# gmongaras/Stable-Diffusion-3-From-Scratch

Hardware: AMD Instinct MI355X
Metric: train images/sec MMDiT-B 256^2 bf16 (higher is better)
Workload: dtype bf16

## Files before the change

### stable-diffusion-3-from-scratch_amd/csrc/attention.hip

```cpp
#include <type_traits>
#include "common.h"

namespace {

constexpr int HD = 64;
constexpr int KT = 64;
constexpr int P144 = 144;
constexpr int P192 = 192;
constexpr float LOG2E = 1.4426950408889634f;
constexpr float LN2 = 0.6931471805599453f;

__device__ __forceinline__ int acc_row(int r, int lane) { return (r & 3) + 8 * (r >> 2) + 4 * (lane >> 5); }

__device__ __forceinline__ bf16x8 pack_frag(const f32x16& p, int h8) {
  u32x4 w;
#pragma unroll
  for (int i = 0; i < 4; i++) w[i] = pack_bf2(p[h8 * 8 + 2 * i], p[h8 * 8 + 2 * i + 1]);
  return __builtin_bit_cast(bf16x8, w);
}

__device__ __forceinline__ bf16x8 tr_frag(const char* tile, int pitch, int rb, int h8, int cb, int lane) {
  const int row = rb + 16 * h8 + 4 * (lane >> 5) + ((lane & 15) >> 2);
  const int col = cb * 32 + 16 * ((lane >> 4) & 1) + (lane & 3) * 4;
  const char* p = tile + row * pitch + col * 2;
  s16x4 lo = lds_tr16(p), hi = lds_tr16(p + 8 * pitch);
  s16x8 r = {lo[0], lo[1], lo[2], lo[3], hi[0], hi[1], hi[2], hi[3]};
  return __builtin_bit_cast(bf16x8, r);
}

__device__ __forceinline__ bf16x8 row_frag(const char* tile, int pitch, int rb, int ks, int lane) {
  return *LDS_PTR(const bf16x8, tile + (rb + (lane & 31)) * pitch + (ks * 16 + (lane >> 5) * 8) * 2);
}

template <int NT> constexpr int tile_chunks() { return (512 + NT - 1) / NT; }
template <int NT>
__device__ __forceinline__ void tile_g2r(u32x4 (&st)[tile_chunks<NT>()], const bf16_t* g, int row0, int nrows_total, int tid) {
#pragma unroll
  for (int i = 0; i < tile_chunks<NT>(); i++) {
    const int c = tid + i * NT, row = c >> 3, kc = c & 7;
    st[i] = (c < 512 && row0 + row < nrows_total) ? *(const u32x4*)(g + (int64_t)(row0 + row) * HD + kc * 8) : (u32x4){0, 0, 0, 0};
  }
}
template <int NT>
__device__ __forceinline__ void tile_r2s(const u32x4 (&st)[tile_chunks<NT>()], char* tile, int pitch, int tid) {
#pragma unroll
  for (int i = 0; i < tile_chunks<NT>(); i++) {
    const int c = tid + i * NT, row = c >> 3, kc = c & 7;
    if (512 % NT == 0 || c < 512) *LDS_PTR(u32x4, tile + row * pitch + kc * 16) = st[i];
  }
}

__device__ __forceinline__ int sw2(int r) { return ((r >> 1) & 7) ^ (((r >> 1) & 1) << 2); }
template <int NT>
__device__ __forceinline__ void tile_r2s_sw(const u32x4 (&st)[tile_chunks<NT>()], char* tile, int tid) {
#pragma unroll
  for (int i = 0; i < tile_chunks<NT>(); i++) {
    const int c = tid + i * NT, row = c >> 3, kc = c & 7;
    if (512 % NT == 0 || c < 512) *LDS_PTR(u32x4, tile + row * 128 + ((kc ^ sw2(row)) << 4)) = st[i];
  }
}
__device__ __forceinline__ bf16x8 row_frag_d(const char* tile, int rb, int ks, int lane) {
  const int r = rb + (lane & 31);
  return *LDS_PTR(const bf16x8, tile + r * 128 + (((ks * 2 + (lane >> 5)) ^ sw2(r)) << 4));
}
__device__ __forceinline__ bf16x8 tr_frag_d(const char* tile, int rb, int h8, int cb, int lane) {
  const int row = rb + 16 * h8 + 4 * (lane >> 5) + ((lane & 15) >> 2);
  const int cbyte = (cb * 32 + 16 * ((lane >> 4) & 1) + (lane & 3) * 4) * 2;
  const char* p0 = tile + row * 128 + ((((cbyte >> 4) ^ sw2(row)) << 4) | (cbyte & 15));
  const char* p1 = tile + (row + 8) * 128 + ((((cbyte >> 4) ^ sw2(row + 8)) << 4) | (cbyte & 15));
  s16x4 lo = lds_tr16(p0), hi = lds_tr16(p1);
  s16x8 r = {lo[0], lo[1], lo[2], lo[3], hi[0], hi[1], hi[2], hi[3]};
  return __builtin_bit_cast(bf16x8, r);
}

__device__ __forceinline__ const bf16_t* tok_ptr(const bf16_t* x_img, const bf16_t* x_txt, int64_t b, int s, int n_img, int n_txt, int D, int h) {
  if (s < n_img) return x_img + ((b * n_img + s) * (int64_t)D + h * HD);
  return x_txt ? x_txt + ((b * n_txt + (s - n_img)) * (int64_t)D + h * HD) : nullptr;
}

__device__ __forceinline__ void map_block(int ntile, int BH, int& tile, int& bh) {
  const int id = blockIdx.x;
  if (BH % 8 == 0) {
    const int xcd = id & 7, j = id >> 3;
    tile = j % ntile;
    bh = (j / ntile) * 8 + xcd;
  } else {
    tile = id % ntile;
    bh = id / ntile;
  }
}

__device__ __forceinline__ float partner32(float x, int lane);
constexpr float QK_RMS_EPS = 1.1920929e-07f;

struct QkFuse {
  const bf16_t* qkv_x; const bf16_t* qkv_c;
  const float* wq_x; const float* wk_x; const float* wq_c; const float* wk_c;
  const float* rcos; const float* rsin;
  bf16_t* dqkv_x; bf16_t* dqkv_c;
  float* dw;
};

constexpr int QK_ROW_F = 68;
constexpr int QK_WAVE_BYTES = 32 * QK_ROW_F * 4;
template <int NW> constexpr int qk_lds_bytes() { return NW * QK_WAVE_BYTES + 128 * 4; }

__device__ __forceinline__ void acc_to_lds(const f32x16 (&acc)[2], float* tile, int lane) {
  float* p = tile + (lane & 31) * QK_ROW_F + 4 * (lane >> 5);
#pragma unroll
  for (int db = 0; db < 2; db++)
#pragma unroll
    for (int g = 0; g < 4; g++)
      *LDS_PTR(f32x4, p + db * 32 + 8 * g) = (f32x4){acc[db][g * 4], acc[db][g * 4 + 1], acc[db][g * 4 + 2], acc[db][g * 4 + 3]};
  __builtin_amdgcn_wave_barrier();
}
__device__ __forceinline__ void acc_to_lds_half(const f32x16 (&acc)[2], float* tile16, int lane, int half) {
  if (((lane & 31) >> 4) == half) {
    float* p = tile16 + (lane & 15) * QK_ROW_F + 4 * (lane >> 5);
#pragma unroll
    for (int db = 0; db < 2; db++)
#pragma unroll
      for (int g = 0; g < 4; g++)
        *LDS_PTR(f32x4, p + db * 32 + 8 * g) = (f32x4){acc[db][g * 4], acc[db][g * 4 + 1], acc[db][g * 4 + 2], acc[db][g * 4 + 3]};
  }
  __builtin_amdgcn_wave_barrier();
}
__device__ __forceinline__ void lds_row8(const float* tile, int r, int c, float (&v)[8]) {
  const f32x4 a = *LDS_PTR(const f32x4, tile + r * QK_ROW_F + 8 * c), b = *LDS_PTR(const f32x4, tile + r * QK_ROW_F + 8 * c + 4);
#pragma unroll
  for (int e = 0; e < 4; e++) { v[e] = a[e]; v[4 + e] = b[e]; }
}
__device__ __forceinline__ void qk_bwd_rows(u32x4 (&xr)[4], int lane, int nvalid, const bf16_t* x0, int64_t pitch) {
  const int c = lane & 7, rsub = lane >> 3;
#pragma unroll
  for (int it = 0; it < 4; it++) xr[it] = __builtin_nontemporal_load((const u32x4*)(x0 + min(it * 8 + rsub, nvalid - 1) * pitch + 8 * c));
}
template <int IT0 = 0, int IT1 = 4>
__device__ __forceinline__ void qk_bwd_tile(const float* tile, float mul, int lane, int nvalid, const bf16_t* x0, bf16_t* o0, int64_t pitch,
                                            const float* w, const float* cs0, const float* sn0, float* sdw, const u32x4* xpre = nullptr) {
  const int c = lane & 7, rsub = lane >> 3;
  float w8[8], dw[8];
  ld8(w + 8 * c, w8);
#pragma unroll
  for (int e = 0; e < 8; e++) dw[e] = 0.f;
  u32x4 xr[4];
  if (xpre) {
#pragma unroll
    for (int it = IT0; it < IT1; it++) xr[it] = xpre[it];
  } else {
#pragma unroll
    for (int it = IT0; it < IT1; it++) xr[it] = __builtin_nontemporal_load((const u32x4*)(x0 + min(it * 8 + rsub, nvalid - 1) * pitch + 8 * c));
  }
  const bool rope = cs0 != nullptr;
  const float* tc = rope ? cs0 : w;
  const float* ts = rope ? sn0 : w;
  auto body = [&](auto full_t) __attribute__((always_inline)) {
    constexpr bool FULL = decltype(full_t)::value;
    float c8[8], s8[8];
    auto request = [&](int it) __attribute__((always_inline)) {
      const int rq = rope ? (FULL ? it * 8 + rsub : min(it * 8 + rsub, nvalid - 1)) : 0;
      ld8(tc + rq * 64 + 8 * c, c8);
      ld8(ts + rq * 64 + 8 * c, s8);
    };
    request(IT0);
#pragma unroll
    for (int it = IT0; it < IT1; it++) {
      const int r = it * 8 + rsub;
      const bool valid = FULL || r < nvalid;
      float dz[8], x[8];
#pragma unroll
      for (int e = 0; e < 4; e++) { x[2 * e] = __builtin_bit_cast(float, xr[it][e] << 16); x[2 * e + 1] = __builtin_bit_cast(float, xr[it][e] & 0xffff0000u); }
      lds_row8(tile, r, c, dz);
#pragma unroll
      for (int e = 0; e < 8; e++) dz[e] *= mul;
      if (rope) {
#pragma unroll
        for (int p = 0; p < 4; p++) {
          const float da = dz[2 * p], dbv = dz[2 * p + 1];
          dz[2 * p] = da * c8[2 * p] + dbv * s8[2 * p + 1];
          dz[2 * p + 1] = dbv * c8[2 * p + 1] - da * s8[2 * p];
        }
      }
      if (it + 1 < IT1) request(it + 1);
      float ss = 0.f;
#pragma unroll
      for (int e = 0; e < 8; e++) ss += x[e] * x[e];
      const float rinv = rsqrtf(sum8(ss) * (1.f / 64.f) + QK_RMS_EPS);
      float dot = 0.f;
#pragma unroll
      for (int e = 0; e < 8; e++) {
        x[e] *= rinv;
        dw[e] += valid ? dz[e] * x[e] : 0.f;
        dz[e] *= w8[e];
        dot += dz[e] * x[e];
      }
      dot = sum8(dot) * (1.f / 64.f);
      float o[8];
#pragma unroll
      for (int e = 0; e < 8; e++) o[e] = rinv * (dz[e] - x[e] * dot);
      if (valid) st8(o0 + r * pitch + 8 * c, o);
    }
  };
  if (nvalid >= 8 * IT1) body(std::integral_constant<bool, true>{});
  else body(std::integral_constant<bool, false>{});
#pragma unroll
  for (int e = 0; e < 8; e++) {
    float v = dw[e];
    v += __shfl_xor(v, 8, 64);
    v += __shfl_xor(v, 16, 64);
    v += __shfl_xor(v, 32, 64);
    if (lane < 8) atomicAdd(&sdw[8 * c + e], v);
  }
}
template <int IT0 = 0, int IT1 = 4>
__device__ __forceinline__ void rows_from_tile(const float* tile, int lane, int nvalid, bf16_t* o0, int64_t pitch) {
  const int c = lane & 7, rsub = lane >> 3;
#pragma unroll
  for (int it = IT0; it < IT1; it++) {
    const int r = it * 8 + rsub;
    float v[8];
    lds_row8(tile, r, c, v);
    if (r < nvalid) st8(o0 + r * pitch + 8 * c, v);
  }
}

template <int NW, bool ORACLE>
__global__ __launch_bounds__(NW * 64) void attn_fwd_kernel(const bf16_t* __restrict__ Q, const bf16_t* __restrict__ K, const bf16_t* __restrict__ V,
                                                            int BH, int H, int S, int n_img, float scale,
                                                            bf16_t* __restrict__ Ox, bf16_t* __restrict__ Oc, float* __restrict__ lse) {
  constexpr int NT = NW * 64;
  __shared__ __attribute__((aligned(16))) char smem[2 * KT * P144 + 2 * KT * P192];
  auto kt = [&](int i) { return smem + i * KT * P144; };
  auto vt = [&](int i) { return smem + 2 * KT * P144 + i * KT * P192; };

  const int tid = threadIdx.x, lane = tid & 63, wave = tid >> 6;
  MMDIT_YOUNG_HALF_PRIO();
  int qtile, bh;
  map_block((S + 32 * NW - 1) / (32 * NW), BH, qtile, bh);
  const int h = bh % H;
  const int64_t b = bh / H;
  const bf16_t* Qb = Q + (int64_t)bh * S * HD;
  const bf16_t* Kb = K + (int64_t)bh * S * HD;
  const bf16_t* Vb = V + (int64_t)bh * S * HD;
// ... 535 lines not shown
  constexpr int NT = NW * 64;
  __shared__ __attribute__((aligned(16))) char smem_static[FUSE ? 16 : 2 * KT * 128 + 2 * KT * 4];
  extern __shared__ __attribute__((aligned(16))) char smem_dyn[];
  char* smem = FUSE ? smem_dyn : smem_static;
  char* qtile = smem;
  char* dotile = smem + KT * 128;
  float* lse_s = (float*)(smem + 2 * KT * 128);
  float* del_s = lse_s + KT;
  const int tid = threadIdx.x, lane = tid & 63, wave = tid >> 6;
  MMDIT_YOUNG_HALF_PRIO();
  int ktile, bh;
  map_block((S + 32 * NW - 1) / (32 * NW), BH, ktile, bh);
  const int h = bh % H;
  const int64_t b = bh / H;
  const bf16_t* Qb = Q + (int64_t)bh * S * HD;
  const bf16_t* Kb = K + (int64_t)bh * S * HD;
  const bf16_t* Vb = V + (int64_t)bh * S * HD;
  const int key = ktile * 32 * NW + wave * 32 + (lane & 31);
  const bool active = ktile * 32 * NW + wave * 32 < S;
  const int keyc = min(key, S - 1);
  const int n_txt = S - n_img, D = H * HD;

  bf16x8 kf[4], vf[4];
#pragma unroll
  for (int ks = 0; ks < 4; ks++) {
    kf[ks] = *(const bf16x8*)(Kb + (int64_t)keyc * HD + ks * 16 + (lane >> 5) * 8);
    vf[ks] = *(const bf16x8*)(Vb + (int64_t)keyc * HD + ks * 16 + (lane >> 5) * 8);
  }
  f32x16 dk[2], dv[2];
#pragma unroll
  for (int db = 0; db < 2; db++)
#pragma unroll
    for (int r = 0; r < 16; r++) { dk[db][r] = 0.f; dv[db][r] = 0.f; }

  const int nq = (S + KT - 1) / KT;
  u32x4 sq[tile_chunks<NT>()], sd[tile_chunks<NT>()];
  float lv = 0.f, dl = 0.f;
  auto request = [&](int jq) {
    tile_g2r<NT>(sq, Qb, jq * KT, S, tid);
#pragma unroll
    for (int i = 0; i < tile_chunks<NT>(); i++) {
      const int c = tid + i * NT, row = c >> 3, kc = c & 7, s = jq * KT + row;
      const bf16_t* p = (c < 512 && s < S) ? tok_ptr(dOx, dOc, b, s, n_img, n_txt, D, h) : nullptr;
      sd[i] = p ? *(const u32x4*)(p + kc * 8) : (u32x4){0, 0, 0, 0};
    }
    lv = 0.f, dl = 0.f;
    if (tid < KT && jq * KT + tid < S) { lv = lse[(int64_t)bh * S + jq * KT + tid]; dl = delta[(int64_t)bh * S + jq * KT + tid]; }
  };
  request(0);
  stamp();
  for (int jq = 0; jq < nq; jq++) {
    __syncthreads();
    stamp();
    tile_r2s_sw<NT>(sq, qtile, tid);
    tile_r2s_sw<NT>(sd, dotile, tid);
    if (tid < KT) { lse_s[tid] = lv * LOG2E; del_s[tid] = dl; }
    stamp();
    __syncthreads();
    stamp();
#ifndef MMDIT_DKV_NO_PREFETCH
    if (jq + 1 < nq) request(jq + 1);
#endif
    if (active) {
#pragma unroll
    for (int qb = 0; qb < 2; qb++) {
      if (jq * KT + qb * 32 >= S) continue;
      f32x16 s, dp;
#pragma unroll
      for (int r = 0; r < 16; r++) { s[r] = 0.f; dp[r] = 0.f; }
#pragma unroll
      for (int ks = 0; ks < 4; ks++) {
        s = __builtin_amdgcn_mfma_f32_32x32x16_bf16(row_frag_d(qtile, qb * 32, ks, lane), kf[ks], s, 0, 0, 0);
        dp = __builtin_amdgcn_mfma_f32_32x32x16_bf16(row_frag_d(dotile, qb * 32, ks, lane), vf[ks], dp, 0, 0, 0);
      }
      if constexpr (TRACE) stamp();
      f32x16 ds;
#pragma unroll
      for (int g = 0; g < 4; g++) {
        const int r0 = qb * 32 + 8 * g + 4 * (lane >> 5);
        const f32x4 l4 = *LDS_PTR(const f32x4, lse_s + r0);
        const f32x4 d4 = *LDS_PTR(const f32x4, del_s + r0);
#pragma unroll
        for (int e = 0; e < 4; e++) {
          const int r = g * 4 + e;
          const float p = fast_exp2(fmaf(s[r], scale * LOG2E, -l4[e]));
          s[r] = p;
          ds[r] = p * (dp[r] - d4[e]);
        }
      }
      if ((jq + 1) * KT > S) {
#pragma unroll
        for (int g = 0; g < 4; g++)
#pragma unroll
          for (int e = 0; e < 4; e++)
            if (jq * KT + qb * 32 + 8 * g + 4 * (lane >> 5) + e >= S) { s[g * 4 + e] = 0.f; ds[g * 4 + e] = 0.f; }
      }
      if constexpr (TRACE) stamp();
#pragma unroll
      for (int h8 = 0; h8 < 2; h8++) {
        const bf16x8 pf = pack_frag(s, h8), dsf = pack_frag(ds, h8);
#pragma unroll
        for (int db = 0; db < 2; db++) {
          dv[db] = __builtin_amdgcn_mfma_f32_32x32x16_bf16(tr_frag_d(dotile, qb * 32, h8, db, lane), pf, dv[db], 0, 0, 0);
          dk[db] = __builtin_amdgcn_mfma_f32_32x32x16_bf16(tr_frag_d(qtile, qb * 32, h8, db, lane), dsf, dk[db], 0, 0, 0);
        }
      }
      if constexpr (TRACE) stamp();
    }
    }
    if constexpr (TRACE) { const int done = !active ? 0 : (jq * KT + 32 >= S ? 1 : 2); for (int i = done * 3; i < 6; i++) stamp(); }
#ifdef MMDIT_DKV_NO_PREFETCH
    if (jq + 1 < nq) request(jq + 1);
#endif
  }
  stamp();
  if constexpr (FUSE) {
    const int k0 = ktile * 32 * NW + wave * 32;
    const bool img = k0 < n_img;
    const int tok0 = img ? k0 : k0 - n_img, nvalid = min(32, (img ? n_img : S) - k0);
    const int64_t pitch = 3 * (int64_t)D, off = (img ? b * n_img + tok0 : b * n_txt + tok0) * pitch + D + h * HD;
    u32x4 xk[4];
    if (active) qk_bwd_rows(xk, lane, nvalid, (img ? F.qkv_x : F.qkv_c) + off, pitch);
    __syncthreads();
    float* sdw = (float*)(smem + NW * QK_WAVE_BYTES);
    if (tid < 128) sdw[tid] = 0.f;
    __syncthreads();
    if (active) {
      bf16_t* ob = (img ? F.dqkv_x : F.dqkv_c) + off;
      float* tile = (float*)(smem + wave * QK_WAVE_BYTES);
      acc_to_lds(dk, tile, lane);
      qk_bwd_tile(tile, scale, lane, nvalid, (img ? F.qkv_x : F.qkv_c) + off, ob, pitch, img ? F.wk_x : F.wk_c,
                  img ? F.rcos + (int64_t)tok0 * 64 : nullptr, img ? F.rsin + (int64_t)tok0 * 64 : nullptr, sdw + (img ? 0 : 64), xk);
      __builtin_amdgcn_wave_barrier();
      acc_to_lds(dv, tile, lane);
      rows_from_tile(tile, lane, nvalid, ob + D, pitch);
    }
    __syncthreads();
    if (tid < 128 && sdw[tid] != 0.f) atomicAdd(F.dw + (tid >> 6) * 128 + 64 + (tid & 63), sdw[tid]);
  } else if (key < S) {
    TG* pk = dK + ((int64_t)bh * S + key) * HD;
    TG* pv = dV + ((int64_t)bh * S + key) * HD;
#pragma unroll
    for (int db = 0; db < 2; db++)
#pragma unroll
      for (int g = 0; g < 4; g++) {
        float k4[4] = {dk[db][g * 4] * scale, dk[db][g * 4 + 1] * scale, dk[db][g * 4 + 2] * scale, dk[db][g * 4 + 3] * scale};
        float v4[4] = {dv[db][g * 4], dv[db][g * 4 + 1], dv[db][g * 4 + 2], dv[db][g * 4 + 3]};
        st4(pk + db * 32 + 8 * g + 4 * (lane >> 5), k4);
        st4(pv + db * 32 + 8 * g + 4 * (lane >> 5), v4);
      }
  }
  if constexpr (TRACE) asm volatile("s_waitcnt vmcnt(0)" ::: "memory");
  stamp();
}

#ifdef MMDIT_PROBES
constexpr int OP_MAXB = 13;
constexpr int OP_DST = 80;
constexpr int OP_DQ_BYTES = OP_MAXB * QK_WAVE_BYTES;
constexpr int OP_R_DST0 = 2 * KT * 128 + 2 * KT * 4;
constexpr int OP_R_BYTES = OP_R_DST0 + 8 * 32 * OP_DST;
constexpr int OP_LDS = OP_DQ_BYTES + OP_R_BYTES + 256 * 4;

__global__ __launch_bounds__(512) void attn_bwd_onepass_kernel(const bf16_t* __restrict__ Q, const bf16_t* __restrict__ K, const bf16_t* __restrict__ V,
                                                               const bf16_t* __restrict__ Ox, const bf16_t* __restrict__ Oc,
                                                               const bf16_t* __restrict__ dOx, const bf16_t* __restrict__ dOc, const float* __restrict__ lse,
                                                               int BH, int H, int S, int n_img, float scale, QkFuse F, int dbg) {
  constexpr int NT = 512;
  extern __shared__ __attribute__((aligned(16))) char smem_dyn[];
  float* dqa = (float*)smem_dyn;
  char* R = smem_dyn + OP_DQ_BYTES;
  char* qtile = R;
  char* dotile = R + KT * 128;
  float* lse_s = (float*)(R + 2 * KT * 128);
  float* del_s = lse_s + KT;
  float* sdw = (float*)(smem_dyn + OP_DQ_BYTES + OP_R_BYTES);
  const int tid = threadIdx.x, lane = tid & 63, wave = __builtin_amdgcn_readfirstlane(tid >> 6);
  char* dst_w = R + OP_R_DST0 + wave * (32 * OP_DST);
  int tile0, bh;
  map_block(1, BH, tile0, bh);
  const int h = bh % H;
  const int64_t b = bh / H;
  const bf16_t* Qb = Q + (int64_t)bh * S * HD;
  const bf16_t* Kb = K + (int64_t)bh * S * HD;
  const bf16_t* Vb = V + (int64_t)bh * S * HD;
  const int n_txt = S - n_img, D = H * HD;
  const int64_t pitch = 3 * (int64_t)D;
  const int nkb = (S + 31) >> 5, nq = (S + KT - 1) / KT;

  for (int i = tid; i < OP_DQ_BYTES / 16; i += NT) *LDS_PTR(f32x4, dqa + 4 * i) = (f32x4){0.f, 0.f, 0.f, 0.f};
  if (tid < 256) sdw[tid] = 0.f;

  u32x4 sq[1], sd[1], so[1];
  float lv = 0.f;
  auto request = [&](int jq) {
    tile_g2r<NT>(sq, Qb, jq * KT, S, tid);
    const int row = tid >> 3, kc = tid & 7, sidx = jq * KT + row;
    const bf16_t* pd = sidx < S ? tok_ptr(dOx, dOc, b, sidx, n_img, n_txt, D, h) : nullptr;
    const bf16_t* po = sidx < S ? tok_ptr(Ox, Oc, b, sidx, n_img, n_txt, D, h) : nullptr;
    sd[0] = pd ? *(const u32x4*)(pd + kc * 8) : (u32x4){0, 0, 0, 0};
    so[0] = (pd && po) ? *(const u32x4*)(po + kc * 8) : (u32x4){0, 0, 0, 0};
    lv = 0.f;
    if (tid < KT && jq * KT + tid < S) lv = lse[(int64_t)bh * S + jq * KT + tid];
  };

#pragma unroll 1
  for (int pass = 0; pass * 8 < nkb; pass++) {
    const int kblk = pass * 8 + wave;
    const bool active = kblk < nkb;
    const int key = kblk * 32 + (lane & 31), keyc = min(key, S - 1);
    const bool ragged_keys = kblk * 32 + 32 > S;
    __syncthreads();
    bf16x8 kf[4], vf[4], kt[2][2];
#pragma unroll
    for (int ks = 0; ks < 4; ks++) {
      kf[ks] = *(const bf16x8*)(Kb + (int64_t)keyc * HD + ks * 16 + (lane >> 5) * 8);
      vf[ks] = *(const bf16x8*)(Vb + (int64_t)keyc * HD + ks * 16 + (lane >> 5) * 8);
    }
    {
      char* kw = R + wave * 4096;
#pragma unroll
      for (int i = 0; i < 4; i++) {
        const int c = lane + 64 * i, row = c >> 3, kc = c & 7;
        const u32x4 v = *(const u32x4*)(Kb + (int64_t)min(kblk * 32 + row, S - 1) * HD + kc * 8);
        *LDS_PTR(u32x4, kw + row * 128 + ((kc ^ sw2(row)) << 4)) = v;
      }
      __builtin_amdgcn_wave_barrier();
#pragma unroll
      for (int h8 = 0; h8 < 2; h8++)
#pragma unroll
        for (int db = 0; db < 2; db++) kt[h8][db] = tr_frag_d(kw, 0, h8, db, lane);
    }
    f32x16 dk[2], dv[2];
#pragma unroll
    for (int db = 0; db < 2; db++)
#pragma unroll
      for (int r = 0; r < 16; r++) { dk[db][r] = 0.f; dv[db][r] = 0.f; }
    request(0);
#pragma unroll 1
    for (int jq = 0; jq < nq; jq++) {
      __syncthreads();
      tile_r2s_sw<NT>(sq, qtile, tid);
      tile_r2s_sw<NT>(sd, dotile, tid);
      {
        float dl = 0.f;
#pragma unroll
        for (int e = 0; e < 4; e++)
          dl += __builtin_bit_cast(float, so[0][e] << 16) * __builtin_bit_cast(float, sd[0][e] << 16) +
                __builtin_bit_cast(float, so[0][e] & 0xffff0000u) * __builtin_bit_cast(float, sd[0][e] & 0xffff0000u);
        dl = sum8(dl);
        if ((tid & 7) == 0) del_s[tid >> 3] = dl;
      }
      if (tid < KT) lse_s[tid] = lv * LOG2E;
      __syncthreads();
      if (jq + 1 < nq) request(jq + 1);
      if (active) {
#pragma unroll 1
        for (int qb = 0; qb < 2; qb++) {
          if (jq * KT + qb * 32 >= S) continue;
          f32x16 sacc, dp;
#pragma unroll
          for (int r = 0; r < 16; r++) { sacc[r] = 0.f; dp[r] = 0.f; }
#pragma unroll
          for (int ks = 0; ks < 4; ks++) {
            sacc = __builtin_amdgcn_mfma_f32_32x32x16_bf16(row_frag_d(qtile, qb * 32, ks, lane), kf[ks], sacc, 0, 0, 0);
            dp = __builtin_amdgcn_mfma_f32_32x32x16_bf16(row_frag_d(dotile, qb * 32, ks, lane), vf[ks], dp, 0, 0, 0);
          }
          f32x16 ds;
#pragma unroll
          for (int g = 0; g < 4; g++) {
            const int r0 = qb * 32 + 8 * g + 4 * (lane >> 5);
            const f32x4 l4 = *LDS_PTR(const f32x4, lse_s + r0);
            const f32x4 d4 = *LDS_PTR(const f32x4, del_s + r0);
#pragma unroll
            for (int e = 0; e < 4; e++) {
              const int r = g * 4 + e;
              const float pe = fast_exp2(fmaf(sacc[r], scale * LOG2E, -l4[e]));
              sacc[r] = pe;
              ds[r] = pe * (dp[r] - d4[e]);
            }
          }
          if ((jq + 1) * KT > S) {
#pragma unroll
            for (int g = 0; g < 4; g++)
#pragma unroll
              for (int e = 0; e < 4; e++)
                if (jq * KT + qb * 32 + 8 * g + 4 * (lane >> 5) + e >= S) { sacc[g * 4 + e] = 0.f; ds[g * 4 + e] = 0.f; }
          }
          if (ragged_keys && key >= S) {
#pragma unroll
            for (int r = 0; r < 16; r++) ds[r] = 0.f;
          }
#pragma unroll
          for (int g = 0; g < 4; g++) {
            const u32x2 w2 = {pack_bf2(ds[g * 4], ds[g * 4 + 1]), pack_bf2(ds[g * 4 + 2], ds[g * 4 + 3])};
            *LDS_PTR(u32x2, dst_w + (lane & 31) * OP_DST + (8 * g + 4 * (lane >> 5)) * 2) = w2;
          }
#pragma unroll
          for (int h8 = 0; h8 < 2; h8++) {
            const bf16x8 pf = pack_frag(sacc, h8), dsf = pack_frag(ds, h8);
#pragma unroll
            for (int db = 0; db < 2; db++) {
              dv[db] = __builtin_amdgcn_mfma_f32_32x32x16_bf16(tr_frag_d(dotile, qb * 32, h8, db, lane), pf, dv[db], 0, 0, 0);
              dk[db] = __builtin_amdgcn_mfma_f32_32x32x16_bf16(tr_frag_d(qtile, qb * 32, h8, db, lane), dsf, dk[db], 0, 0, 0);
            }
          }
// ... 191 lines not shown
        for (int w = 0; w < 2; w++) {
          to4[h8][db][w] = lds_tr16(tq + h8 * 16 * 128 + KT * 128 + troff[db][w]);
          tq4[h8][db][w] = lds_tr16(tq + h8 * 16 * 128 + troff[db][w]);
        }
  };
  auto mfma_sdp = [&]() {
#ifdef MMDIT_DKV_NOMFMA
#pragma unroll
    for (int ks = 0; ks < 4; ks++) { s[ks] = (float)fq[ks][0]; dp[ks] = (float)fo[ks][0]; }
    return;
#endif
#pragma unroll
    for (int ks = 0; ks < 4; ks++) {
      s = __builtin_amdgcn_mfma_f32_32x32x16_bf16(fq[ks], kf[ks], ks == 0 ? zero16 : s, 0, 0, 0);
      dp = __builtin_amdgcn_mfma_f32_32x32x16_bf16(fo[ks], vf[ks], ks == 0 ? zero16 : dp, 0, 0, 0);
    }
  };
  auto softmax_bwd = [&](int bq) {
    const char* tl = tile_of(bq) + 2 * KT * 128;
    const int qb = bq & 1, hi = lane >> 5;
    f32x16 ds;
    f32x4 lq[4], dq4[4];
#pragma unroll
    for (int g = 0; g < 4; g++) {
      const int r0 = qb * 32 + 8 * g + 4 * hi;
      lq[g] = *LDS_PTR(const f32x4, tl + r0 * 4);
      dq4[g] = *LDS_PTR(const f32x4, tl + KT * 4 + r0 * 4);
    }
    __builtin_amdgcn_sched_barrier(0);
#pragma unroll
    for (int g = 0; g < 4; g++) {
      const f32x4 l4 = lq[g], d4 = dq4[g];
#pragma unroll
      for (int e = 0; e < 4; e += 2) {
        const int r = g * 4 + e;
        const f32x2 sv = {s[r], s[r + 1]}, dpv = {dp[r], dp[r + 1]};
        const f32x2 nl = (f32x2){l4[e], l4[e + 1]} * (f32x2){-LOG2E, -LOG2E};
        const f32x2 t = __builtin_elementwise_fma(sv, (f32x2){c, c}, nl);
#ifdef MMDIT_DKV_NOEXP
        const f32x2 pv = t;
#else
        const f32x2 pv = {fast_exp2(t[0]), fast_exp2(t[1])};
#endif
        const f32x2 dsv = pv * (dpv - (f32x2){d4[e], d4[e + 1]});
        s[r] = pv[0]; s[r + 1] = pv[1];
        ds[r] = dsv[0]; ds[r + 1] = dsv[1];
      }
    }
    if ((bq + 1) * 32 > S) {
#pragma unroll
      for (int g = 0; g < 4; g++)
#pragma unroll
        for (int e = 0; e < 4; e++)
          if (bq * 32 + 8 * g + 4 * hi + e >= S) { s[g * 4 + e] = 0.f; ds[g * 4 + e] = 0.f; }
    }
#pragma unroll
    for (int h8 = 0; h8 < 2; h8++) { pf[h8] = pack_frag(s, h8); dsf[h8] = pack_frag(ds, h8); }
  };
  auto mfma_dkv = [&]() {
#ifdef MMDIT_DKV_NOMFMA
#pragma unroll
    for (int h8 = 0; h8 < 2; h8++)
#pragma unroll
      for (int db = 0; db < 2; db++) { dv[db][h8] += (float)to4[h8][db][0][0] + (float)to4[h8][db][1][0] + (float)pf[h8][0]; dk[db][h8] += (float)tq4[h8][db][0][0] + (float)tq4[h8][db][1][0] + (float)dsf[h8][0]; }
    return;
#endif
#pragma unroll
    for (int h8 = 0; h8 < 2; h8++)
#pragma unroll
      for (int db = 0; db < 2; db++) {
        const s16x4 olo = to4[h8][db][0], ohi = to4[h8][db][1], qlo = tq4[h8][db][0], qhi = tq4[h8][db][1];
        const s16x8 of = {olo[0], olo[1], olo[2], olo[3], ohi[0], ohi[1], ohi[2], ohi[3]};
        const s16x8 qf = {qlo[0], qlo[1], qlo[2], qlo[3], qhi[0], qhi[1], qhi[2], qhi[3]};
        dv[db] = __builtin_amdgcn_mfma_f32_32x32x16_bf16(__builtin_bit_cast(bf16x8, of), pf[h8], dv[db], 0, 0, 0);
        dk[db] = __builtin_amdgcn_mfma_f32_32x32x16_bf16(__builtin_bit_cast(bf16x8, qf), dsf[h8], dk[db], 0, 0, 0);
      }
  };
  auto bar = [&]() { asm volatile("s_waitcnt lgkmcnt(0)" ::: "memory"); __builtin_amdgcn_s_barrier(); };

  wait_tiles(min(2, nq - 1));
  asm volatile("" : "+v"(kf[0]), "+v"(kf[1]), "+v"(kf[2]), "+v"(kf[3]), "+v"(vf[0]), "+v"(vf[1]), "+v"(vf[2]), "+v"(vf[3]));
  bar();
  if (active) { read_rows(0); mfma_sdp(); read_tr(0); }
  stamp();
#ifndef MMDIT_DKV_NOSTAGGER
  if (grp == 1) bar();
#endif
  for (int bq = 0; bq < nblk; bq++) {
    if (active) softmax_bwd(bq);
    stamp();
#ifdef MMDIT_DKV_NODMA
    if (bq == 0) wait_tiles(0);
#else
    if (!(bq & 1)) wait_tiles(max(0, min(1, nq - 2 - (bq >> 1))));
#endif
    __builtin_amdgcn_s_barrier();
    stamp();
    if (active && bq + 1 < nblk) read_rows(bq + 1);
    const int t2 = (bq >> 1) + DKV_ST - 1;
#ifndef MMDIT_DKV_NODMA
    if (!(bq & 1) && t2 < nq) issue(t2);
#endif
    stamp();
    if (active) {
      __builtin_amdgcn_sched_barrier(0);
      mfma_dkv();
      __builtin_amdgcn_sched_barrier(0);
      stamp();
      if (bq + 1 < nblk) { read_tr(bq + 1); __builtin_amdgcn_sched_barrier(0); mfma_sdp(); }
    } else stamp();
    __builtin_amdgcn_s_barrier();
    stamp();
  }
#ifndef MMDIT_DKV_NOSTAGGER
  if (grp == 0) bar();
#endif
  __syncthreads();
  if constexpr (FUSE) {
    float* sdw = (float*)(smem + NW * QK_WAVE_BYTES);
    if (tid < 128) sdw[tid] = 0.f;
    __syncthreads();
    if (active) {
      const int k0 = ktile * 32 * NW + wave * 32;
      const bool img = k0 < n_img;
      const int tok0 = img ? k0 : k0 - n_img, nvalid = min(32, (img ? n_img : S) - k0);
      const int64_t pitch = 3 * (int64_t)D, off = (img ? b * n_img + tok0 : b * n_txt + tok0) * pitch + D + h * HD;
      bf16_t* ob = (img ? F.dqkv_x : F.dqkv_c) + off;
      float* tile = (float*)(smem + wave * QK_WAVE_BYTES);
      acc_to_lds(dk, tile, lane);
      qk_bwd_tile(tile, scale, lane, nvalid, (img ? F.qkv_x : F.qkv_c) + off, ob, pitch, img ? F.wk_x : F.wk_c,
                  img ? F.rcos + (int64_t)tok0 * 64 : nullptr, img ? F.rsin + (int64_t)tok0 * 64 : nullptr, sdw + (img ? 0 : 64));
      __builtin_amdgcn_wave_barrier();
      acc_to_lds(dv, tile, lane);
      rows_from_tile(tile, lane, nvalid, ob + D, pitch);
    }
    __syncthreads();
    if (tid < 128 && sdw[tid] != 0.f) atomicAdd(F.dw + (tid >> 6) * 128 + 64 + (tid & 63), sdw[tid]);
  } else if (key < S) {
    TG* pk = dK + ((int64_t)bh * S + key) * HD;
    TG* pv = dV + ((int64_t)bh * S + key) * HD;
#pragma unroll
    for (int db = 0; db < 2; db++)
#pragma unroll
      for (int g = 0; g < 4; g++) {
        float k4[4] = {dk[db][g * 4] * scale, dk[db][g * 4 + 1] * scale, dk[db][g * 4 + 2] * scale, dk[db][g * 4 + 3] * scale};
        float v4[4] = {dv[db][g * 4], dv[db][g * 4 + 1], dv[db][g * 4 + 2], dv[db][g * 4 + 3]};
        st4(pk + db * 32 + 8 * g + 4 * (lane >> 5), k4);
        st4(pv + db * 32 + 8 * g + 4 * (lane >> 5), v4);
      }
  }
}
#endif

int attn_waves(int S) {
  (void)S;
#ifdef MMDIT_PROBES
  static const char* e = getenv("MMDIT_ATTN_NW");
  if (e) return atoi(e);
#endif
  return 8;
}

}

extern "C" int mmdit_attn_fwd(const void* Q, const void* K, const void* V, int batch, int heads, int S, int n_img, float scale, int mode,
                              void* Ox, void* Oc, float* lse, mmdit_stream_t stream) {
  MMDIT_CHECK_ARG(Q && K && V && Ox && lse && batch > 0 && heads > 0 && S > 0 && n_img > 0 && n_img <= S);
  MMDIT_CHECK_ARG(Oc || n_img == S);
  hipStream_t s = (hipStream_t)stream;
  const int nw = attn_waves(S);
#define MMDIT_FWD(NW, OR) hipLaunchKernelGGL((attn_fwd_kernel<NW, OR>), dim3(((S + 32 * NW - 1) / (32 * NW)) * batch * heads), dim3(NW * 64), 0, s, (const bf16_t*)Q, (const bf16_t*)K, \
                                             (const bf16_t*)V, batch * heads, heads, S, n_img, scale, (bf16_t*)Ox, (bf16_t*)Oc, lse)
  if (mode == 1) MMDIT_FWD(2, true);
  else if (mode != 0) return MMDIT_ERR_ARG;
#ifdef MMDIT_PROBES
  else if ((getenv("MMDIT_ATTN_DMA") && atoi(getenv("MMDIT_ATTN_DMA")) == 0) || getenv("MMDIT_ATTN_NW")) {
    if (nw == 8) MMDIT_FWD(8, false);
    else if (nw == 7) MMDIT_FWD(7, false);
    else if (nw == 6) MMDIT_FWD(6, false);
    else if (nw == 4) MMDIT_FWD(4, false);
    else MMDIT_FWD(2, false);
  }
#endif
#define MMDIT_FWD_DMA(NW, NS) hipLaunchKernelGGL((attn_fwd_dma_kernel<0, false, NW, NS>), dim3(((S + 32 * NW - 1) / (32 * NW)) * batch * heads), dim3(64 * NW), 0, s, (const bf16_t*)Q, \
                                                (const bf16_t*)K, (const bf16_t*)V, batch * heads, heads, S, n_img, scale, (bf16_t*)Ox, (bf16_t*)Oc, lse)
#ifdef MMDIT_PROBES
  else if (mmdit_exp_env("MMDIT_ATTN_FWD_GEO") && atoi(mmdit_exp_env("MMDIT_ATTN_FWD_GEO")) != 84) {
    switch (atoi(mmdit_exp_env("MMDIT_ATTN_FWD_GEO"))) {
      case 83: MMDIT_FWD_DMA(8, 3); break;
      case 44: MMDIT_FWD_DMA(4, 4); break;
      case 43: MMDIT_FWD_DMA(4, 3); break;
      case 42: MMDIT_FWD_DMA(4, 2); break;
      default: return MMDIT_ERR_ARG;
    }
  }
#endif
  else MMDIT_FWD_DMA(8, 4);
#undef MMDIT_FWD_DMA
#undef MMDIT_FWD
  return mmdit_launch_status();
}


extern "C" int mmdit_attn_fwd_mx(const void* Q, const void* K, const void* V, int batch, int heads, int S, int n_img, float scale,
                                 void* Ox_fp8, void* Oc_fp8, void* scales_x, void* scales_c, mmdit_stream_t stream) {
  MMDIT_CHECK_ARG(Q && K && V && Ox_fp8 && scales_x && batch > 0 && heads > 0 && S > 0 && n_img > 0 && n_img <= S);
  MMDIT_CHECK_ARG((Oc_fp8 && scales_c) || n_img == S);
  hipLaunchKernelGGL((attn_fwd_dma_kernel<0, true>), dim3(((S + 255) / 256) * batch * heads), dim3(512), 0, (hipStream_t)stream, (const bf16_t*)Q, (const bf16_t*)K,
                     (const bf16_t*)V, batch * heads, heads, S, n_img, scale, (bf16_t*)Ox_fp8, (bf16_t*)Oc_fp8, nullptr, (unsigned char*)scales_x, (unsigned char*)scales_c);
  return mmdit_launch_status();
}

#ifdef MMDIT_PROBES
extern "C" int mmdit_probe_attn_fwd_dbg(const void* Q, const void* K, const void* V, int batch, int heads, int S, int n_img, float scale,
                                        void* Ox, void* Oc, float* lse, int dbg, mmdit_stream_t stream) {
#define MMDIT_DBG(D) case D: hipLaunchKernelGGL(attn_fwd_dma_kernel<D>, dim3(((S + 255) / 256) * batch * heads), dim3(512), 0, (hipStream_t)stream, (const bf16_t*)Q, \
                                                 (const bf16_t*)K, (const bf16_t*)V, batch * heads, heads, S, n_img, scale, (bf16_t*)Ox, (bf16_t*)Oc, lse); break;
  switch (dbg) {
    MMDIT_DBG(0) MMDIT_DBG(1) MMDIT_DBG(2) MMDIT_DBG(4) MMDIT_DBG(8) MMDIT_DBG(16) MMDIT_DBG(32) MMDIT_DBG(33) MMDIT_DBG(6) MMDIT_DBG(39) MMDIT_DBG(24) MMDIT_DBG(57) MMDIT_DBG(63) MMDIT_DBG(64) MMDIT_DBG(191) MMDIT_DBG(128)
    default: return MMDIT_ERR_ARG;
  }
#undef MMDIT_DBG
  return mmdit_launch_status();
}

#endif

#ifdef MMDIT_PROBES
extern "C" int mmdit_probe_attn_bwd_dkv_trace(const void* Q, const void* K, const void* V, const void* dOx, const void* dOc, const float* lse, const float* delta,
                                              int batch, int heads, int S, int n_img, float scale, void* dK, void* dV, void* trace, mmdit_stream_t stream) {
  hipLaunchKernelGGL((attn_bwd_dkv_kernel<8, bf16_t, false, true>), dim3(((S + 255) / 256) * batch * heads), dim3(512), 0, (hipStream_t)stream, (const bf16_t*)Q, (const bf16_t*)K,
                     (const bf16_t*)V, (const bf16_t*)dOx, (const bf16_t*)dOc, lse, delta, batch * heads, heads, S, n_img, scale, (bf16_t*)dK, (bf16_t*)dV, QkFuse(),
                     (unsigned long long*)trace);
  return mmdit_launch_status();
}
#endif

#ifdef MMDIT_PROBES
extern "C" int mmdit_probe_attn_bwd_dkv_dp_trace(const void* Q, const void* K, const void* V, const void* dOx, const void* dOc, const float* lse, const float* delta,
                                                 int batch, int heads, int S, int n_img, float scale, void* dK, void* dV, void* trace, mmdit_stream_t stream) {
  static unsigned long long raised = 0;
  if (!mmdit_device_once(raised)) {
    hipError_t e = hipFuncSetAttribute(reinterpret_cast<const void*>(&attn_bwd_dkv_dp_kernel<bf16_t, false, true>), hipFuncAttributeMaxDynamicSharedMemorySize, dkv_lds_bytes<false>());
    if (e != hipSuccess) return (int)e;
    mmdit_device_mark(raised);
  }
  hipLaunchKernelGGL((attn_bwd_dkv_dp_kernel<bf16_t, false, true>), dim3(((S + 255) / 256) * batch * heads), dim3(512), dkv_lds_bytes<false>(), (hipStream_t)stream, (const bf16_t*)Q,
                     (const bf16_t*)K, (const bf16_t*)V, (const bf16_t*)dOx, (const bf16_t*)dOc, lse, delta, batch * heads, heads, S, n_img, scale, (bf16_t*)dK, (bf16_t*)dV, QkFuse(),
                     (unsigned long long*)trace);
  return mmdit_launch_status();
}
#endif

extern "C" int mmdit_attn_bwd_qk(const void* Q, const void* K, const void* V, const void* Ox, const void* Oc, const void* dOx, const void* dOc,
                                 const float* lse, float* delta, int batch, int heads, int S, int n_img, float scale,
                                 const void* qkv_x, const void* qkv_c, const float* wq_x, const float* wk_x, const float* wq_c, const float* wk_c,
                                 const float* rope_cos, const float* rope_sin, void* dqkv_x, void* dqkv_c, float* dw, mmdit_stream_t stream) {
  MMDIT_CHECK_ARG(Q && K && V && Ox && dOx && lse && delta && batch > 0 && heads > 0 && S > 0 && n_img > 0 && n_img <= S);
  MMDIT_CHECK_ARG(Oc || n_img == S);
  MMDIT_CHECK_ARG(qkv_x && wq_x && wk_x && rope_cos && rope_sin && dqkv_x && dw && (n_img == S || (qkv_c && wq_c && wk_c && dqkv_c)));
  if (n_img % 32) return MMDIT_ERR_SHAPE;
  const QkFuse F{(const bf16_t*)qkv_x, (const bf16_t*)qkv_c, wq_x, wk_x, wq_c, wk_c, rope_cos, rope_sin, (bf16_t*)dqkv_x, (bf16_t*)dqkv_c, dw};
  hipStream_t s = (hipStream_t)stream;
  const dim3 grid(((S + 255) / 256) * batch * heads);
  constexpr int lds = qk_lds_bytes<8>();
  static unsigned long long raised = 0;
  if (!mmdit_device_once(raised)) {
    hipError_t e = hipFuncSetAttribute(reinterpret_cast<const void*>(&attn_bwd_dq_kernel<8, bf16_t, true>), hipFuncAttributeMaxDynamicSharedMemorySize, lds);
    if (e == hipSuccess) e = hipFuncSetAttribute(reinterpret_cast<const void*>(&attn_bwd_dkv_kernel<8, bf16_t, true>), hipFuncAttributeMaxDynamicSharedMemorySize, lds);
#ifdef MMDIT_PROBES
    if (e == hipSuccess) e = hipFuncSetAttribute(reinterpret_cast<const void*>(&attn_bwd_dkv_dp_kernel<bf16_t, true>), hipFuncAttributeMaxDynamicSharedMemorySize, dkv_lds_bytes<true>());
#endif
    if (e != hipSuccess) return (int)e;
    mmdit_device_mark(raised);
  }
#ifdef MMDIT_PROBES
  if (S <= 32 * OP_MAXB && mmdit_exp_env("MMDIT_ATTN_ONEPASS") && atoi(mmdit_exp_env("MMDIT_ATTN_ONEPASS")) == 1) {
    static unsigned long long raised1 = 0;
    if (!mmdit_device_once(raised1)) {
      hipError_t e = hipFuncSetAttribute(reinterpret_cast<const void*>(&attn_bwd_onepass_kernel), hipFuncAttributeMaxDynamicSharedMemorySize, OP_LDS);
      if (e != hipSuccess) return (int)e;
      mmdit_device_mark(raised1);
    }
    hipLaunchKernelGGL(attn_bwd_onepass_kernel, dim3(batch * heads), dim3(512), OP_LDS, s, (const bf16_t*)Q, (const bf16_t*)K, (const bf16_t*)V, (const bf16_t*)Ox,
                       (const bf16_t*)Oc, (const bf16_t*)dOx, (const bf16_t*)dOc, lse, batch * heads, heads, S, n_img, scale, F,
                       mmdit_exp_env("MMDIT_OP_DBG") ? atoi(mmdit_exp_env("MMDIT_OP_DBG")) : 0);
    return mmdit_launch_status();
  }
#endif
  hipLaunchKernelGGL((attn_bwd_dq_kernel<8, bf16_t, true>), grid, dim3(512), lds, s, (const bf16_t*)Q, (const bf16_t*)K, (const bf16_t*)V, (const bf16_t*)Ox,
                     (const bf16_t*)Oc, (const bf16_t*)dOx, (const bf16_t*)dOc, lse, delta, batch * heads, heads, S, n_img, scale, (bf16_t*)nullptr, F);
#ifdef MMDIT_PROBES
  if (mmdit_exp_env("MMDIT_ATTN_DKV_DP") && atoi(mmdit_exp_env("MMDIT_ATTN_DKV_DP")) == 1 && (dOc || n_img == S)) {
    hipLaunchKernelGGL((attn_bwd_dkv_dp_kernel<bf16_t, true>), grid, dim3(512), dkv_lds_bytes<true>(), s, (const bf16_t*)Q, (const bf16_t*)K, (const bf16_t*)V, (const bf16_t*)dOx,
                       (const bf16_t*)dOc, lse, delta, batch * heads, heads, S, n_img, scale, (bf16_t*)nullptr, (bf16_t*)nullptr, F);
    return mmdit_launch_status();
  }
#endif
  hipLaunchKernelGGL((attn_bwd_dkv_kernel<8, bf16_t, true>), grid, dim3(512), lds, s, (const bf16_t*)Q, (const bf16_t*)K, (const bf16_t*)V, (const bf16_t*)dOx,
                     (const bf16_t*)dOc, lse, delta, batch * heads, heads, S, n_img, scale, (bf16_t*)nullptr, (bf16_t*)nullptr, F);
  return mmdit_launch_status();
}

extern "C" int mmdit_attn_bwd(const void* Q, const void* K, const void* V, const void* Ox, const void* Oc, const void* dOx, const void* dOc,
                              const float* lse, float* delta, int batch, int heads, int S, int n_img, float scale,
                              void* dQ, void* dK, void* dV, int dq_dtype, mmdit_stream_t stream) {
  MMDIT_CHECK_ARG(Q && K && V && Ox && dOx && lse && delta && dQ && dK && dV && batch > 0 && heads > 0 && S > 0 && n_img > 0 && n_img <= S);
  MMDIT_CHECK_ARG(Oc || n_img == S);
  hipStream_t s = (hipStream_t)stream;
  const int nw = attn_waves(S);
#define MMDIT_DKV(NW, TG) hipLaunchKernelGGL((attn_bwd_dkv_kernel<NW, TG>), dim3(((S + 32 * NW - 1) / (32 * NW)) * batch * heads), dim3(NW * 64), 0, s, (const bf16_t*)Q, (const bf16_t*)K, \
                                             (const bf16_t*)V, (const bf16_t*)dOx, (const bf16_t*)dOc, lse, delta, batch * heads, heads, S, n_img, scale, (TG*)dK, (TG*)dV)
#define MMDIT_DQ(NW, TG) hipLaunchKernelGGL((attn_bwd_dq_kernel<NW, TG>), dim3(((S + 32 * NW - 1) / (32 * NW)) * batch * heads), dim3(NW * 64), 0, s, (const bf16_t*)Q, (const bf16_t*)K, \
                                            (const bf16_t*)V, (const bf16_t*)Ox, (const bf16_t*)Oc, (const bf16_t*)dOx, (const bf16_t*)dOc, lse, delta, batch * heads, heads, S, n_img, scale, (TG*)dQ)
  if (dq_dtype == MMDIT_BF16) {
#ifdef MMDIT_PROBES
    if (nw == 7) { MMDIT_DQ(7, bf16_t); MMDIT_DKV(7, bf16_t); }
    else if (nw == 6) { MMDIT_DQ(6, bf16_t); MMDIT_DKV(6, bf16_t); }
    else if (nw == 4) { MMDIT_DQ(4, bf16_t); MMDIT_DKV(4, bf16_t); }
    else if (nw == 2) { MMDIT_DQ(2, bf16_t); MMDIT_DKV(2, bf16_t); }
    else
#endif
    { MMDIT_DQ(8, bf16_t); MMDIT_DKV(8, bf16_t); }
  } else if (dq_dtype == MMDIT_F32) {
    MMDIT_DQ(2, float);
    MMDIT_DKV(2, float);
  } else return MMDIT_ERR_DTYPE;
#undef MMDIT_DQ
#undef MMDIT_DKV
  return mmdit_launch_status();
}
```

Before: 2434.

## Add persistent dK/dV attention backward kernel that prefetches the next tile during epilogue

Adds a persistent-grid version of the attention backward dK/dV kernel. Each block loops over (key tile, head) work items, sized by CU count times occupancy. While the current item's epilogue runs (fused QK-norm/RoPE backward or plain stores), it starts loading the next item's K/V and first Q/dO tile, so the epilogue and tail latency are overlapped and the per-block launch overhead is removed. It is on by default, can be disabled via env, and adds a launch-time occupancy query plus more complex control flow.

```diff
diff --git a/stable-diffusion-3-from-scratch_amd/csrc/attention.hip b/stable-diffusion-3-from-scratch_amd/csrc/attention.hip
--- a/stable-diffusion-3-from-scratch_amd/csrc/attention.hip
+++ b/stable-diffusion-3-from-scratch_amd/csrc/attention.hip
@@ -78,8 +78,7 @@
   return x_txt ? x_txt + ((b * n_txt + (s - n_img)) * (int64_t)D + h * HD) : nullptr;
 }
 
-__device__ __forceinline__ void map_block(int ntile, int BH, int& tile, int& bh) {
-  const int id = blockIdx.x;
+__device__ __forceinline__ void map_item(int id, int ntile, int BH, int& tile, int& bh) {
   if (BH % 8 == 0) {
     const int xcd = id & 7, j = id >> 3;
     tile = j % ntile;
@@ -89,6 +88,7 @@
     bh = id / ntile;
   }
 }
+__device__ __forceinline__ void map_block(int ntile, int BH, int& tile, int& bh) { map_item(blockIdx.x, ntile, BH, tile, bh); }
 
 __device__ __forceinline__ float partner32(float x, int lane);
 constexpr float QK_RMS_EPS = 1.1920929e-07f;
@@ -930,6 +930,175 @@
   }
   if constexpr (TRACE) asm volatile("s_waitcnt vmcnt(0)" ::: "memory");
   stamp();
+}
+
+template <bool FUSE> constexpr int dkvp_lds_bytes() { return FUSE ? 2 * 8 * QK_WAVE_BYTES + 128 * 4 : 2 * KT * 128 + 2 * KT * 4; }
+
+template <typename TG, bool FUSE>
+__global__ __launch_bounds__(512) void attn_bwd_dkv_pers_kernel(const bf16_t* __restrict__ Q, const bf16_t* __restrict__ K, const bf16_t* __restrict__ V,
+                                                                const bf16_t* __restrict__ dOx, const bf16_t* __restrict__ dOc,
+                                                                const float* __restrict__ lse, const float* __restrict__ delta,
+                                                                int BH, int H, int S, int n_img, float scale, TG* __restrict__ dK, TG* __restrict__ dV, QkFuse F = QkFuse()) {
+  constexpr int NW = 8, NT = NW * 64;
+  extern __shared__ __attribute__((aligned(16))) char smem[];
+  char* qtile = smem;
+  char* dotile = smem + KT * 128;
+  float* lse_s = (float*)(smem + 2 * KT * 128);
+  float* del_s = lse_s + KT;
+  float* sdw = (float*)(smem + 2 * NW * QK_WAVE_BYTES);
+  const int tid = threadIdx.x, lane = tid & 63, wave = tid >> 6;
+  MMDIT_YOUNG_HALF_PRIO();
+  const int ntile = (S + 32 * NW - 1) / (32 * NW), nitems = ntile * BH;
+  const int n_txt = S - n_img, D = H * HD;
+  const int nq = (S + KT - 1) / KT;
+  if (FUSE && tid < 128) sdw[tid] = 0.f;
+
+  int item = blockIdx.x, ktile, bh, h, key, keyc;
+  int64_t b;
+  bool active;
+  const bf16_t *Qb, *Kb, *Vb;
+  auto setup = [&]() {
+    map_item(item, ntile, BH, ktile, bh);
+    h = bh % H;
+    b = bh / H;
+    Qb = Q + (int64_t)bh * S * HD;
+    Kb = K + (int64_t)bh * S * HD;
+    Vb = V + (int64_t)bh * S * HD;
+    key = ktile * 32 * NW + wave * 32 + (lane & 31);
+    active = ktile * 32 * NW + wave * 32 < S;
+    keyc = min(key, S - 1);
+  };
+  bf16x8 kf[4], vf[4];
+  auto load_kv = [&]() {
+#pragma unroll
+    for (int ks = 0; ks < 4; ks++) {
+      kf[ks] = *(const bf16x8*)(Kb + (int64_t)keyc * HD + ks * 16 + (lane >> 5) * 8);
+      vf[ks] = *(const bf16x8*)(Vb + (int64_t)keyc * HD + ks * 16 + (lane >> 5) * 8);
+    }
+  };
+  u32x4 sq[1], sd[1];
+  float lv = 0.f, dl = 0.f;
+  auto request = [&](int jq) {
+    int t = tid;
+    asm volatile("" : "+v"(t));
+    const int crow = t >> 3, ccol = (t & 7) * 8, s = jq * KT + crow;
+    sq[0] = s < S ? *(const u32x4*)(Qb + (uint32_t)(s * HD + ccol)) : (u32x4){0, 0, 0, 0};
+    const bf16_t* dbase = s < n_img ? dOx + (b * n_img * (int64_t)D + h * HD) : (dOc ? dOc + (b * n_txt * (int64_t)D + h * HD) : nullptr);
+    const uint32_t doff = (uint32_t)((s < n_img ? s : s - n_img) * D + ccol);
+    sd[0] = (s < S && dbase) ? *(const u32x4*)(dbase + doff) : (u32x4){0, 0, 0, 0};
+    lv = 0.f, dl = 0.f;
+    if (t < KT && jq * KT + t < S) {
+      const uint32_t r = (uint32_t)(jq * KT + t);
+      lv = (lse + (int64_t)bh * S)[r];
+      dl = (delta + (int64_t)bh * S)[r];
+    }
+  };
+  static_assert(tile_chunks<NT>() == 1, "one chunk of each tile per thread");
+  setup();
+  load_kv();
+  request(0);
+
+  for (;;) {
+    f32x16 dk[2], dv[2];
+#pragma unroll
+    for (int db = 0; db < 2; db++)
+#pragma unroll
+      for (int r = 0; r < 16; r++) { dk[db][r] = 0.f; dv[db][r] = 0.f; }
+    for (int jq = 0; jq < nq; jq++) {
+      __syncthreads();
+      tile_r2s_sw<NT>(sq, qtile, tid);
+      tile_r2s_sw<NT>(sd, dotile, tid);
+      if (tid < KT) { lse_s[tid] = lv * LOG2E; del_s[tid] = dl; }
+      __syncthreads();
+      if (jq + 1 < nq) request(jq + 1);
+      if (active) {
+#pragma unroll
+      for (int qb = 0; qb < 2; qb++) {
+        if (jq * KT + qb * 32 >= S) continue;
+        f32x16 s, dp;
+#pragma unroll
+        for (int r = 0; r < 16; r++) { s[r] = 0.f; dp[r] = 0.f; }
+#pragma unroll
+        for (int ks = 0; ks < 4; ks++) {
+          s = __builtin_amdgcn_mfma_f32_32x32x16_bf16(row_frag_d(qtile, qb * 32, ks, lane), kf[ks], s, 0, 0, 0);
+          dp = __builtin_amdgcn_mfma_f32_32x32x16_bf16(row_frag_d(dotile, qb * 32, ks, lane), vf[ks], dp, 0, 0, 0);
+        }
+        f32x16 ds;
+#pragma unroll
+        for (int g = 0; g < 4; g++) {
+          const int r0 = qb * 32 + 8 * g + 4 * (lane >> 5);
+          const f32x4 l4 = *LDS_PTR(const f32x4, lse_s + r0);
+          const f32x4 d4 = *LDS_PTR(const f32x4, del_s + r0);
+#pragma unroll
+          for (int e = 0; e < 4; e++) {
+            const int r = g * 4 + e;
+            const float p = fast_exp2(fmaf(s[r], scale * LOG2E, -l4[e]));
+            s[r] = p;
+            ds[r] = p * (dp[r] - d4[e]);
+          }
+        }
+        if ((jq + 1) * KT > S) {
+#pragma unroll
+          for (int g = 0; g < 4; g++)
+#pragma unroll
+            for (int e = 0; e < 4; e++)
+              if (jq * KT + qb * 32 + 8 * g + 4 * (lane >> 5) + e >= S) { s[g * 4 + e] = 0.f; ds[g * 4 + e] = 0.f; }
+        }
+#pragma unroll
+        for (int h8 = 0; h8 < 2; h8++) {
+          const bf16x8 pf = pack_frag(s, h8), dsf = pack_frag(ds, h8);
+#pragma unroll
+          for (int db = 0; db < 2; db++) {
+            dv[db] = __builtin_amdgcn_mfma_f32_32x32x16_bf16(tr_frag_d(dotile, qb * 32, h8, db, lane), pf, dv[db], 0, 0, 0);
+            dk[db] = __builtin_amdgcn_mfma_f32_32x32x16_bf16(tr_frag_d(qtile, qb * 32, h8, db, lane), dsf, dk[db], 0, 0, 0);
+          }
+        }
+      }
+      }
+    }
+    const bool cur_active = active;
+    const int next = item + gridDim.x;
+    if constexpr (FUSE) {
+      const int k0 = ktile * 32 * NW + wave * 32;
+      const bool img = k0 < n_img;
+      const int tok0 = img ? k0 : k0 - n_img, nvalid = min(32, (img ? n_img : S) - k0);
+      const int64_t pitch = 3 * (int64_t)D, off = (img ? b * n_img + tok0 : b * n_txt + tok0) * pitch + D + h * HD;
+      if (next < nitems) { item = next; setup(); load_kv(); request(0); }
+      u32x4 xk[4];
+      if (cur_active) qk_bwd_rows(xk, lane, nvalid, (img ? F.qkv_x : F.qkv_c) + off, pitch);
+      __syncthreads();
+      float* tk = (float*)(smem + wave * QK_WAVE_BYTES);
+      float* tv = (float*)(smem + (NW + wave) * QK_WAVE_BYTES);
+      if (cur_active) { acc_to_lds(dk, tk, lane); acc_to_lds(dv, tv, lane); }
+      if (cur_active) {
+        bf16_t* ob = (img ? F.dqkv_x : F.dqkv_c) + off;
+        qk_bwd_tile(tk, scale, lane, nvalid, (img ? F.qkv_x : F.qkv_c) + off, ob, pitch, img ? F.wk_x : F.wk_c,
+                    img ? F.rcos + (int64_t)tok0 * 64 : nullptr, img ? F.rsin + (int64_t)tok0 * 64 : nullptr, sdw + (img ? 0 : 64), xk);
+        rows_from_tile(tv, lane, nvalid, ob + D, pitch);
+      }
+    } else {
+      TG* pk = dK + ((int64_t)bh * S + key) * HD;
+      TG* pv = dV + ((int64_t)bh * S + key) * HD;
+      const bool store = key < S;
+      if (next < nitems) { item = next; setup(); load_kv(); request(0); }
+      if (store) {
+#pragma unroll
+        for (int db = 0; db < 2; db++)
+#pragma unroll
+          for (int g = 0; g < 4; g++) {
+            float k4[4] = {dk[db][g * 4] * scale, dk[db][g * 4 + 1] * scale, dk[db][g * 4 + 2] * scale, dk[db][g * 4 + 3] * scale};
+            float v4[4] = {dv[db][g * 4], dv[db][g * 4 + 1], dv[db][g * 4 + 2], dv[db][g * 4 + 3]};
+            st4(pk + db * 32 + 8 * g + 4 * (lane >> 5), k4);
+            st4(pv + db * 32 + 8 * g + 4 * (lane >> 5), v4);
+          }
+      }
+    }
+    if (next >= nitems) break;
+  }
+  if constexpr (FUSE) {
+    __syncthreads();
+    if (tid < 128 && sdw[tid] != 0.f) atomicAdd(F.dw + (tid >> 6) * 128 + 64 + (tid & 63), sdw[tid]);
+  }
 }
 
 #ifdef MMDIT_PROBES
@@ -1427,6 +1596,31 @@
 }
 #endif
 
+bool dkv_persistent() {
+  const char* e = mmdit_exp_env("MMDIT_ATTN_DKV_PERSIST");
+  return !(e && atoi(e) == 0);
+}
+template <typename TG, bool FUSE>
+int dkv_pers_launch(const void* Q, const void* K, const void* V, const void* dOx, const void* dOc, const float* lse, const float* delta,
+                    int batch, int heads, int S, int n_img, float scale, void* dK, void* dV, const QkFuse& F, hipStream_t s) {
+  const void* fn = reinterpret_cast<const void*>(&attn_bwd_dkv_pers_kernel<TG, FUSE>);
+  constexpr int lds = dkvp_lds_bytes<FUSE>();
+  static unsigned long long raised = 0;
+  static int occ[64];
+  if (!mmdit_device_once(raised)) {
+    hipError_t e = hipFuncSetAttribute(fn, hipFuncAttributeMaxDynamicSharedMemorySize, lds);
+    int n = 0;
+    if (e == hipSuccess) e = hipOccupancyMaxActiveBlocksPerMultiprocessor(&n, fn, 512, lds);
+    if (e != hipSuccess) return (int)e;
+    occ[mmdit_current_device()] = n > 0 ? n : 1;
+    mmdit_device_mark(raised);
+  }
+  const long items = (long)((S + 255) / 256) * batch * heads, slots = (long)mmdit_get_cu_budget() * occ[mmdit_current_device()];
+  hipLaunchKernelGGL((attn_bwd_dkv_pers_kernel<TG, FUSE>), dim3((unsigned)(items < slots ? items : slots)), dim3(512), lds, s, (const bf16_t*)Q, (const bf16_t*)K,
+                     (const bf16_t*)V, (const bf16_t*)dOx, (const bf16_t*)dOc, lse, delta, batch * heads, heads, S, n_img, scale, (TG*)dK, (TG*)dV, F);
+  return mmdit_launch_status();
+}
+
 int attn_waves(int S) {
   (void)S;
 #ifdef MMDIT_PROBES
@@ -1572,6 +1766,10 @@
     return mmdit_launch_status();
   }
 #endif
+  if (dkv_persistent()) {
+    const int e = mmdit_launch_status();
+    return e ? e : dkv_pers_launch<bf16_t, true>(Q, K, V, dOx, dOc, lse, delta, batch, heads, S, n_img, scale, nullptr, nullptr, F, s);
+  }
   hipLaunchKernelGGL((attn_bwd_dkv_kernel<8, bf16_t, true>), grid, dim3(512), lds, s, (const bf16_t*)Q, (const bf16_t*)K, (const bf16_t*)V, (const bf16_t*)dOx,
                      (const bf16_t*)dOc, lse, delta, batch * heads, heads, S, n_img, scale, (bf16_t*)nullptr, (bf16_t*)nullptr, F);
   return mmdit_launch_status();
@@ -1596,7 +1794,14 @@
     else if (nw == 2) { MMDIT_DQ(2, bf16_t); MMDIT_DKV(2, bf16_t); }
     else
 #endif
-    { MMDIT_DQ(8, bf16_t); MMDIT_DKV(8, bf16_t); }
+    {
+      MMDIT_DQ(8, bf16_t);
+      if (dkv_persistent()) {
+        const int e = mmdit_launch_status();
+        return e ? e : dkv_pers_launch<bf16_t, false>(Q, K, V, dOx, dOc, lse, delta, batch, heads, S, n_img, scale, dK, dV, QkFuse(), s);
+      }
+      MMDIT_DKV(8, bf16_t);
+    }
   } else if (dq_dtype == MMDIT_F32) {
     MMDIT_DQ(2, float);
     MMDIT_DKV(2, float);
```

New measurement: 2440, median of 6. About the same (+0.3%).
